# PacificBiosciences/pb-StarPhase

Hardware: AMD Instinct MI355X
Metric: HiFi reads/sec diplotyped (HLA+CYP2D6) (higher is better)
Workload: dtype int32; 1 GPU; BASELINE configs[1] + configs[2] as ONE sample per step: HLA-A/-B 10000 HiFi reads vs IMGT/HLA v0.14.1 (11,199 DNA alleles) + CYP2D6 2000 targeted reads (39 templates), the six configs[2] scenarios in turn; a new sample uploaded every step; reads -> diplotypes; hla_reads=10000, cyp2d6_reads=2000, cyp2d6_lanes=6, hla_lanes=2, cyp2d6_consensus=launch pairs

## Files before the change

### pb-starphase_amd/csrc/sp_api.hip

```cpp
#include "sp_internal.h"
#include <algorithm>
#include <thread>
#include <atomic>
#include <cstring>
#include <new>
#include <unistd.h>

extern "C" {

int32_t sp_abi_version(void) { return SP_ABI_VERSION; }

int32_t sp_device_count(int32_t* count) {
    int n = 0;
    hipError_t e = hipGetDeviceCount(&n);
    if (count) *count = (e == hipSuccess) ? n : 0;
    return e == hipSuccess ? SP_OK : SP_ERR_NO_DEVICE;
}

int32_t sp_ctx_create(int32_t device, void* stream, sp_ctx** out) {
    if (!out) return SP_ERR_INVALID_ARG;
    *out = nullptr;
    static std::atomic<int> effective{-1};
    bool by_library = false;
    if (effective.load() < 0) {
// ... 62 lines not shown
    if (ctx->ev_fork) hipEventDestroy(ctx->ev_fork);
    if (ctx->ev_join) hipEventDestroy(ctx->ev_join);
    hipStreamSynchronize(ctx->stream);
    for (sp_seqset* s : ctx->live_sets) {
        for (void* p : { (void*)s->d_words, (void*)s->d_nplane, (void*)s->d_word_off, (void*)s->d_len, (void*)s->d_kcode, (void*)s->d_kpos, (void*)s->d_koff }) if (p) ctx->dev_cap.erase(p);
        s->ctx = nullptr;
    }
    for (auto& kv : ctx->dev_cap) (void)hipFree(kv.first);
    if (ctx->scratch) hipFree(ctx->scratch);
    for (auto& kv : ctx->pool) if (kv.second.first) hipFree(kv.second.first);
    for (auto& kv : ctx->host_pool) if (kv.second.first) hipHostFree(kv.second.first);
    sp_profile_flush(ctx);
    for (hipEvent_t e : ctx->prof_free) hipEventDestroy(e);
    if (ctx->ev0) hipEventDestroy(ctx->ev0);
    if (ctx->ev1) hipEventDestroy(ctx->ev1);
    if (ctx->own_stream && ctx->stream) hipStreamDestroy(ctx->stream);
    delete ctx;
}

}
sp_ctx* sp_ctx_helper(sp_ctx* ctx, int i) {
    if (i < 0 || i > 6) return nullptr;
    if (!ctx->helper[i] && sp_ctx_create(ctx->device, nullptr, &ctx->helper[i]) != SP_OK) ctx->helper[i] = nullptr;
    if (ctx->helper[i]) { ctx->helper[i]->profiling = ctx->profiling; ctx->helper[i]->k5_block_pairs = ctx->k5_block_pairs; ctx->helper[i]->k8_persistent = ctx->k8_persistent; ctx->helper[i]->k8_side_orders = ctx->k8_side_orders; ctx->helper[i]->k8_compound = ctx->k8_compound; ctx->helper[i]->k8_side_max_blocks = ctx->k8_side_max_blocks; ctx->helper[i]->mm2_rescore = ctx->mm2_rescore; ctx->helper[i]->profile_rescore_counts = ctx->profile_rescore_counts; ctx->helper[i]->k1_best_n = ctx->k1_best_n; }
    return ctx->helper[i];
}
void sp_profile_merge(sp_ctx* into, sp_ctx* from) {
    sp_profile_flush(from);
    for (auto& kv : from->prof) { ProfileEntry& e = into->prof[kv.first]; e.ms += kv.second.ms; e.launches += kv.second.launches; e.cells += kv.second.cells; }
    from->prof.clear();
}
extern "C" {

int32_t sp_struct_size(const char* name) {
    if (!name) return -1;
#define SP_SZ(T) if (std::strcmp(name, #T) == 0) return (int32_t)sizeof(T);
    SP_SZ(sp_ctx_info)
    SP_SZ(sp_pair)
    SP_SZ(sp_aln)
    SP_SZ(sp_hla_db_desc)
    SP_SZ(sp_hla_realign)
    SP_SZ(sp_k1_seed_hit)
    SP_SZ(sp_hla_best)
    SP_SZ(sp_chain_problem)
    SP_SZ(sp_chain_result)
    SP_SZ(sp_region_hit)
    SP_SZ(sp_cyp_problem)
// ... 36 lines not shown
    SP_SZ(sp_starphase_batch_timing)
    SP_SZ(sp_hla_alleles_stats)
    SP_SZ(sp_hla_cfg_mapping)
    SP_SZ(sp_hla_cfg_gene)
    SP_SZ(sp_pileup_col)
    SP_SZ(sp_support_summary)
    SP_SZ(sp_support_entry)
#undef SP_SZ
    return -1;
}

const char* sp_last_error(const sp_ctx* ctx) { return ctx ? ctx->err.c_str() : "null context"; }

int32_t sp_ctx_synchronize(sp_ctx* ctx) {
    if (!ctx) return SP_ERR_INVALID_ARG;
    SP_HIP_CHECK(ctx, hipStreamSynchronize(ctx->stream));
    return SP_OK;
}

int32_t sp_ctx_set_option(sp_ctx* ctx, const char* name, int64_t value) {
    if (!ctx || !name) return SP_ERR_INVALID_ARG;
    if (std::strcmp(name, "hla_split_genes") == 0) { ctx->split_genes = value != 0; return SP_OK; }
    if (std::strcmp(name, "k1_best_n") == 0) { if (value < 0 || value > 8) return sp_fail(ctx, SP_ERR_INVALID_ARG, "sp_ctx_set_option: k1_best_n is 0..8"); ctx->k1_best_n = (int)value; for (sp_ctx* h : ctx->helper) if (h) h->k1_best_n = ctx->k1_best_n; return SP_OK; }
    if (std::strcmp(name, "profile_rescore_counts") == 0) { ctx->profile_rescore_counts = value != 0; for (sp_ctx* h : ctx->helper) if (h) h->profile_rescore_counts = ctx->profile_rescore_counts; return SP_OK; }
    if (std::strcmp(name, "mm2_rescore") == 0) { ctx->mm2_rescore = (int)value; for (sp_ctx* h : ctx->helper) if (h) h->mm2_rescore = ctx->mm2_rescore; return SP_OK; }
    if (std::strcmp(name, "k8_side_orders") == 0) { if (value < 0 || value > 3) return sp_fail(ctx, SP_ERR_INVALID_ARG, "sp_ctx_set_option: k8_side_orders is 0 .. 3"); ctx->k8_side_orders = (int)value; for (sp_ctx* h : ctx->helper) if (h) h->k8_side_orders = ctx->k8_side_orders; return SP_OK; }
    if (std::strcmp(name, "k8_compound") == 0) { ctx->k8_compound = (int)value; for (sp_ctx* h : ctx->helper) if (h) h->k8_compound = ctx->k8_compound; return SP_OK; }
    if (std::strcmp(name, "k8_side_max_blocks") == 0) { if (value < 0) return sp_fail(ctx, SP_ERR_INVALID_ARG, "sp_ctx_set_option: k8_side_max_blocks >= 0"); ctx->k8_side_max_blocks = (int)value; for (sp_ctx* h : ctx->helper) if (h) h->k8_side_max_blocks = ctx->k8_side_max_blocks; return SP_OK; }
    if (std::strcmp(name, "k8_persistent") == 0) { if (value < 0 || value > 2) return sp_fail(ctx, SP_ERR_INVALID_ARG, "sp_ctx_set_option: k8_persistent is 0 (never), 1 (whenever a batch fits) or 2 (the library decides)"); ctx->k8_persistent = (int)value; ctx->k8_persist_backoff = 0; ctx->k8_persist_failures = 0; for (sp_ctx* h : ctx->helper) if (h) h->k8_persistent = ctx->k8_persistent; return SP_OK; }
    if (std::strcmp(name, "cons_retry_ladder") == 0) { ctx->cons_retry_ladder = value != 0; for (sp_ctx* h : ctx->helper) if (h) h->cons_retry_ladder = ctx->cons_retry_ladder; return SP_OK; }
    if (std::strcmp(name, "k5_block_pairs") == 0) { if (value < 0 || value > (1 << 20)) return sp_fail(ctx, SP_ERR_INVALID_ARG, "sp_ctx_set_option: k5_block_pairs is 0..1048576"); ctx->k5_block_pairs = (int)value; for (sp_ctx* h : ctx->helper) if (h) h->k5_block_pairs = ctx->k5_block_pairs; return SP_OK; }
    if (std::strcmp(name, "cyp_cohort_min_group") == 0) { if (value < 1 || value > 64) return sp_fail(ctx, SP_ERR_INVALID_ARG, "sp_ctx_set_option: cyp_cohort_min_group is 1..64"); ctx->cyp_cohort_min_group = (int)value; return SP_OK; }
    if (std::strcmp(name, "cyp_cohort_streams") == 0) { if (value < 1 || value > 8) return sp_fail(ctx, SP_ERR_INVALID_ARG, "sp_ctx_set_option: cyp_cohort_streams is 1..8"); ctx->cyp_cohort_streams = (int)value; return SP_OK; }
    if (std::strcmp(name, "hla_split_streams") == 0) { if (value < 1 || value > 4) return sp_fail(ctx, SP_ERR_INVALID_ARG, "sp_ctx_set_option: hla_split_streams is 1..4"); ctx->split_streams = (int)value; return SP_OK; }
    return sp_fail(ctx, SP_ERR_INVALID_ARG, std::string("sp_ctx_set_option: unknown option ") + name);
}

int32_t sp_profile_reset(sp_ctx* ctx) {
    if (!ctx) return SP_ERR_INVALID_ARG;
    for (sp_ctx* h : ctx->helper) if (h) sp_profile_reset(h);
    sp_profile_flush(ctx); ctx->prof.clear();
    unsigned long long* c = sp_counters(ctx);
    if (c) { hipSetDevice(ctx->device); hipMemsetAsync(c, 0, SPC_N * sizeof(unsigned long long), ctx->stream); }
    return SP_OK;
}

// ... 200 lines not shown
    ctx->dev_cap[p] = want;
    return p;
}
void sp_dev_release(sp_ctx* ctx, void* p) {
    if (!p) return;
    constexpr size_t MAX_BYTES = (size_t)2 << 30, MAX_BUFFERS = 4096;
    {
        std::lock_guard<std::mutex> g(ctx->dev_cache_mu);
        auto it = ctx->dev_cap.find(p);
        if (it == ctx->dev_cap.end()) { (void)hipFree(p); return; }
        if (ctx->dev_cache.size() < MAX_BUFFERS && ctx->dev_cache_bytes + it->second <= MAX_BYTES) { ctx->dev_cache.emplace(it->second, p); ctx->dev_cache_bytes += it->second; return; }
        ctx->dev_cap.erase(it);
    }
    (void)hipFree(p);
}
extern "C" {

int32_t sp_seqset_skipped(const sp_seqset* s, uint32_t* n_skipped) { if (!s || !n_skipped) return SP_ERR_INVALID_ARG; *n_skipped = s->n_skipped; return SP_OK; }

void sp_seqset_free(sp_seqset* s) {
    if (!s) return;
    if (s->ctx) hipSetDevice(s->ctx->device);
    if (s->up) { (void)upload_finish(s); }
    if (s->ctx) {
        (void)hipStreamSynchronize(s->ctx->stream);
        { std::lock_guard<std::mutex> g(s->ctx->dev_cache_mu); s->ctx->live_sets.erase(s); }
        sp_dev_release(s->ctx, s->d_words); sp_dev_release(s->ctx, s->d_nplane); sp_dev_release(s->ctx, s->d_word_off); sp_dev_release(s->ctx, s->d_len);
        sp_dev_release(s->ctx, s->d_kcode); sp_dev_release(s->ctx, s->d_kpos); sp_dev_release(s->ctx, s->d_koff);
    } else {
        if (s->d_words) hipFree(s->d_words);
        if (s->d_nplane) hipFree(s->d_nplane);
        if (s->d_word_off) hipFree(s->d_word_off);
        if (s->d_len) hipFree(s->d_len);
        if (s->d_kcode) hipFree(s->d_kcode);
        if (s->d_kpos) hipFree(s->d_kpos);
        if (s->d_koff) hipFree(s->d_koff);
    }
    delete s;
}

int32_t sp_seqset_count(const sp_seqset* s, uint32_t* n) { if (!s || !n) return SP_ERR_INVALID_ARG; *n = s->n; return SP_OK; }
int32_t sp_seqset_length(const sp_seqset* s, uint32_t idx, uint32_t* len) {
    if (!s || !len || idx >= s->n) return SP_ERR_INVALID_ARG;
    *len = (uint32_t)s->h_len[idx]; return SP_OK;
}

// ... 171 lines not shown
    hipMemcpy(s->d_koff, koff.data(), koff.size() * 8, hipMemcpyHostToDevice);
    s->has_index = true;
    return SP_OK;
}

extern "C" {

int32_t sp_anchor_batch_topk(sp_ctx* ctx, const sp_seqset* A, const sp_seqset* B,
                             const uint32_t* a_idx, const uint32_t* b_idx, uint64_t n_pairs, int32_t topk,
                             int32_t* diag_out, int32_t* votes_out) {
    if (!ctx || !A || !B || (n_pairs && (!a_idx || !b_idx || !diag_out || !votes_out))) return SP_ERR_INVALID_ARG;
    if (topk < 1 || topk > 8) return sp_fail(ctx, SP_ERR_INVALID_ARG, "anchor: topk must be 1..8");
    if (n_pairs == 0) return SP_OK;
    hipSetDevice(ctx->device);
    for (uint64_t i = 0; i < n_pairs; ++i) if (a_idx[i] >= A->n || b_idx[i] >= B->n) return sp_fail(ctx, SP_ERR_INVALID_ARG, "anchor: index out of range");
    int rc = sp_seqset_build_index(ctx, const_cast<sp_seqset*>(A));
    if (rc) return rc;
    const size_t nb = n_pairs * 4, nbk = nb * (size_t)topk;
    uint32_t* d_a = (uint32_t*)sp_pool(ctx, "anchor_a", nb); uint32_t* d_b = (uint32_t*)sp_pool(ctx, "anchor_b", nb);
    int32_t* d_d = (int32_t*)sp_pool(ctx, "anchor_d", nbk); int32_t* d_v = (int32_t*)sp_pool(ctx, "anchor_v", nbk);
    if (!d_a || !d_b || !d_d || !d_v) return sp_fail(ctx, SP_ERR_OUT_OF_MEMORY, "anchor buffers");
    hipMemcpyAsync(d_a, a_idx, nb, hipMemcpyHostToDevice, ctx->stream);
    hipMemcpyAsync(d_b, b_idx, nb, hipMemcpyHostToDevice, ctx->stream);
    rc = sp_launch_anchor(ctx, A, B, d_a, d_b, n_pairs, d_d, d_v, topk);
    if (rc == SP_OK) {
        hipMemcpyAsync(diag_out, d_d, nbk, hipMemcpyDeviceToHost, ctx->stream);
        hipMemcpyAsync(votes_out, d_v, nbk, hipMemcpyDeviceToHost, ctx->stream);
        if (hipStreamSynchronize(ctx->stream) != hipSuccess) rc = sp_fail(ctx, SP_ERR_HIP, "anchor: stream sync failed");
    }
    return rc;
}

int32_t sp_anchor_batch(sp_ctx* ctx, const sp_seqset* A, const sp_seqset* B,
                        const uint32_t* a_idx, const uint32_t* b_idx, uint64_t n_pairs,
                        int32_t* diag_out, int32_t* votes_out) {
    return sp_anchor_batch_topk(ctx, A, B, a_idx, b_idx, n_pairs, 1, diag_out, votes_out);
}

int32_t sp_align_batch(sp_ctx* ctx, const sp_seqset* A, const sp_seqset* B,
                       const sp_pair* pairs, uint64_t n_pairs,
                       sp_aln* out, uint32_t* events, uint32_t events_stride) {
    if (!ctx || !A || !B || (n_pairs && (!pairs || !out))) return SP_ERR_INVALID_ARG;
    if (events && (events_stride == 0 || events_stride > SP_MAX_ED)) return sp_fail(ctx, SP_ERR_INVALID_ARG, "align: events_stride must be 1..SP_MAX_ED");
    if (n_pairs == 0) return SP_OK;
    hipSetDevice(ctx->device);
    std::vector<CellDesc> cells(n_pairs);
    for (uint64_t i = 0; i < n_pairs; ++i) {
// ... 24 lines not shown
```

### pb-starphase_amd/csrc/sp_cyp.hip

```cpp
#include "sp_internal.h"
#include <system_error>
#include <thread>
#include <atomic>
#include <memory>
#include <map>
#include "sp_json.h"
#include "sp_wfa.hip.h"
#include <algorithm>
#include <cmath>
#include <cstring>
#include <numeric>
#include <string>
#include <vector>

namespace {

inline bool t_is_cyp2d(int t) { return t == SP_CYP_CYP2D6 || t == SP_CYP_CYP2D7 || t == SP_CYP_DELETION || t == SP_CYP_HYBRID; }
inline bool t_is_rep(int t) { return t == SP_CYP_REP6 || t == SP_CYP_REP7; }
inline bool t_is_reported(int t) { return t == SP_CYP_CYP2D6 || t == SP_CYP_DELETION || t == SP_CYP_HYBRID; }
inline bool t_allowed(int t) { return t != SP_CYP_UNKNOWN && t != SP_CYP_FALSE_ALLELE; }
inline bool t_normalizing(int t, bool all) { return all ? t_is_cyp2d(t) : t == SP_CYP_CYP2D6; }
inline bool t_head(int t, bool all) {
    if (t == SP_CYP_REP6 || t == SP_CYP_DELETION) return true;
    if (t == SP_CYP_CYP2D6 || t == SP_CYP_HYBRID) return t_normalizing(t, all);
// ... 591 lines not shown
    if (e != hipSuccess) return sp_fail(ctx, SP_ERR_HIP, std::string("cyp placements: ") + hipGetErrorString(e));
    return SP_OK;
}

__global__ void cyp_all_pairs_kernel(uint32_t nA, uint64_t n_pairs, uint32_t* __restrict__ a_idx, uint32_t* __restrict__ b_idx) {
    const uint64_t i = (uint64_t)blockIdx.x * blockDim.x + threadIdx.x;
    if (i >= n_pairs) return;
    a_idx[i] = (uint32_t)(i % nA); b_idx[i] = (uint32_t)(i / nA);
}
static int cyp_align_all_pinned(sp_ctx* ctx, const sp_seqset* A, const sp_seqset* B, int topk, double frac_cap, const char* prof, sp_aln** out, int32_t** diag_out, int32_t** votes_out) {
    const uint64_t nA = A->n, n_pairs = nA * (uint64_t)B->n, n_cells = n_pairs * (uint64_t)topk;
    *out = nullptr; *diag_out = nullptr; *votes_out = nullptr;
    if (n_pairs == 0) return SP_OK;
    int rc = sp_seqset_build_index(ctx, const_cast<sp_seqset*>(A));
    if (rc) return rc;
    uint32_t* d_a = (uint32_t*)sp_pool(ctx, "cyp_a", n_pairs * 4); uint32_t* d_b = (uint32_t*)sp_pool(ctx, "cyp_b", n_pairs * 4);
    int32_t* d_d = (int32_t*)sp_pool(ctx, "cyp_d", n_cells * 4); int32_t* d_v = (int32_t*)sp_pool(ctx, "cyp_v", n_cells * 4);
    CellDesc* d_cells = (CellDesc*)sp_pool(ctx, "cyp_cells", n_cells * sizeof(CellDesc));
    sp_aln* d_alns = (sp_aln*)sp_pool(ctx, "cyp_alns", n_cells * sizeof(sp_aln));
    sp_aln* h_alns = (sp_aln*)sp_host_pool(ctx, "k3_alns_host", n_cells * sizeof(sp_aln));
    int32_t* h_d = (int32_t*)sp_host_pool(ctx, "k3_diag_host", n_cells * 4); int32_t* h_v = (int32_t*)sp_host_pool(ctx, "k3_votes_host", n_cells * 4);
    if (!d_a || !d_b || !d_d || !d_v || !d_cells || !d_alns || !h_alns || !h_d || !h_v) return sp_fail(ctx, SP_ERR_OUT_OF_MEMORY, "cyp placement buffers");
    hipLaunchKernelGGL(cyp_all_pairs_kernel, dim3((unsigned)((n_pairs + 255) / 256)), dim3(256), 0, ctx->stream, (uint32_t)nA, n_pairs, d_a, d_b);
    rc = sp_launch_anchor(ctx, A, B, d_a, d_b, n_pairs, d_d, d_v, topk, "anchor", (uint32_t)nA);
    if (rc) return rc;
    hipLaunchKernelGGL(cyp_build_cells_kernel, dim3((unsigned)((n_cells + 255) / 256)), dim3(256), 0, ctx->stream, d_a, d_b, d_d, d_v, n_pairs, topk, CYP_MIN_VOTES, A->d_len, frac_cap, d_cells);
    rc = sp_launch_cells(ctx, A, B, d_cells, n_cells, d_alns, nullptr, 0, prof, 0);
    if (rc) return rc;
    (void)hipMemcpyAsync(h_alns, d_alns, n_cells * sizeof(sp_aln), hipMemcpyDeviceToHost, ctx->stream);
    (void)hipMemcpyAsync(h_d, d_d, n_cells * 4, hipMemcpyDeviceToHost, ctx->stream);
    (void)hipMemcpyAsync(h_v, d_v, n_cells * 4, hipMemcpyDeviceToHost, ctx->stream);
    hipError_t e = hipStreamSynchronize(ctx->stream);
    if (e != hipSuccess) return sp_fail(ctx, SP_ERR_HIP, std::string("cyp placements: ") + hipGetErrorString(e));
    *out = h_alns; *diag_out = h_d; *votes_out = h_v;
    return SP_OK;
}

static int cyp_align_all(sp_ctx* ctx, const sp_seqset* A, const sp_seqset* B, int topk, double frac_cap, int retry_wide, const char* prof, std::vector<sp_aln>& out,
                         std::vector<int32_t>* diag_out = nullptr, std::vector<int32_t>* votes_out = nullptr) {
    const uint64_t nA = A->n, nB = B->n, n_pairs = nA * nB;
    std::vector<uint32_t> ai(n_pairs), bi(n_pairs);
    for (uint64_t b = 0; b < nB; ++b) for (uint64_t a = 0; a < nA; ++a) { ai[b * nA + a] = (uint32_t)a; bi[b * nA + a] = (uint32_t)b; }
    return cyp_align_pairs(ctx, A, B, ai, bi, (uint32_t)nA, topk, frac_cap, retry_wide, prof, out, diag_out, votes_out);
}

static inline double cyp_score(int seq_len, int nm, int unmapped, bool penalize) {
    const int len = penalize ? seq_len : seq_len - unmapped;
// ... 1303 lines not shown
                                             sp_cyp_region_variants* region_variants) {
    return spi_cyp_diplotype_mappings(ctx, pr, reads, call, consensus, cons_cap, region_variants, nullptr);
}

extern "C" int32_t sp_cyp_diplotype_mappings(sp_ctx* ctx, const sp_cyp_problem* pr, const sp_seqset* reads, sp_cyp_call* call, char* consensus, uint32_t cons_cap,
                                             sp_cyp_region_variants* region_variants, sp_cyp_read_mapping* mappings, uint64_t cap, uint64_t* n_mappings) {
    if (!n_mappings || (cap && !mappings)) return ctx ? sp_fail(ctx, SP_ERR_INVALID_ARG, "sp_cyp_diplotype_mappings: null argument") : SP_ERR_INVALID_ARG;
    std::vector<sp_cyp_read_mapping> all;
    const int32_t rc = spi_cyp_diplotype_mappings(ctx, pr, reads, call, consensus, cons_cap, region_variants, &all);
    *n_mappings = all.size();
    if (rc != SP_OK) return rc;
    std::copy(all.begin(), all.begin() + std::min<uint64_t>(cap, all.size()), mappings);
    return all.size() > cap ? sp_fail(ctx, SP_ERR_CAPACITY, "sp_cyp_diplotype_mappings: more read mappings than cap") : SP_OK;
}

int32_t spi_cyp_diplotype_cohort_mappings(sp_ctx* ctx, const sp_cyp_problem* pr, uint32_t n_samples, const sp_seqset* const* reads, sp_cyp_call* calls,
                                          char* consensus, uint32_t cons_cap, sp_cyp_region_variants* region_variants,
                                          std::vector<sp_cyp_read_mapping>* mappings, int32_t* sample_rc) {
    if (!ctx) return SP_ERR_INVALID_ARG;
    if (!pr || (n_samples && (!reads || !calls))) return sp_fail(ctx, SP_ERR_INVALID_ARG, "sp_cyp_diplotype_cohort: null argument");
    for (uint32_t i = 0; i < n_samples; ++i) if (!reads[i]) return sp_fail(ctx, SP_ERR_INVALID_ARG, "sp_cyp_diplotype_cohort: null read set");
    if (n_samples == 0) return SP_OK;
    if (pr->templates) { const int rc0 = sp_seqset_build_index(ctx, const_cast<sp_seqset*>(pr->templates)); if (rc0 != SP_OK) return rc0; }
    const uint32_t stream_cap = ctx->k8_persistent ? std::min(ctx->cyp_cohort_streams, 4) : ctx->cyp_cohort_streams;
    int n_parts = ctx->split_genes ? (int)std::min<uint32_t>(std::max<uint32_t>(1, n_samples / (uint32_t)ctx->cyp_cohort_min_group), stream_cap) : 1;
    sp_ctx* on[8] = { ctx, nullptr, nullptr, nullptr, nullptr, nullptr, nullptr, nullptr };
    for (int x = 1; x < n_parts; ++x) { on[x] = sp_ctx_helper(ctx, x - 1); if (!on[x]) { n_parts = x; break; } }
    std::vector<int32_t> rcs(n_samples, SP_OK); std::vector<int> where(n_samples, 0);
    std::atomic<uint32_t> next(0);
    const uint32_t group = std::min<uint32_t>(64, std::max<uint32_t>(1, (n_samples + (uint32_t)n_parts - 1) / (uint32_t)n_parts));
    auto work = [&](int x) {
        sp_ctx* c = on[x];
        (void)hipSetDevice(c->device);
        for (;;) {
            const uint32_t first = next.fetch_add(group);
            if (first >= n_samples) break;
            const uint32_t n = std::min<uint32_t>(group, n_samples - first);
            std::vector<std::unique_ptr<CypMid>> mids(n);
            std::vector<sp_priority_job> jobs; std::vector<uint32_t> job_of;
            try {
                std::vector<std::vector<sp_region_hit>> group_hits; int32_t rc_regions = SP_OK;
                sp_seqset view; std::vector<uint32_t> view_first;
                const bool viewed = pr->templates && pr->template_type && cyp_group_view(c, reads + first, n, "cypg", view, view_first, rc_regions);
                const bool searched = viewed && (rc_regions != SP_OK || cyp_group_regions(c, pr, view, view_first, n, group_hits, rc_regions));
                for (uint32_t k = 0; k < n; ++k) {
                    const uint32_t i = first + k;
// ... 255 lines not shown
```

### pb-starphase_amd/csrc/sp_internal.h

```cpp
#pragma once
#include <hip/hip_runtime.h>
#include <stdint.h>
#include <string>
#include <vector>
#include <chrono>
#include <set>
#include <mutex>
#include <map>
#include "../../include/starphase_hip.h"

#define SP_NEG        (-(1 << 28))
#define SP_SEQ_PAD_WORDS 512
#define SP_LDS_TAIL    288
#define SP_WAVE       64
#define SP_MAXOCC     4
#define SP_CELL_NONE  0xFFFFFFFFu
#define SP_PEAK_SPREAD   48
#define SP_PEAK_SUPPRESS 128

struct SeqSetView {
    const uint32_t* words;
    const uint32_t* nplane;
    const uint64_t* word_off;
    const int32_t*  len;
// ... 4 lines not shown
    const uint32_t* code;
    const int32_t*  pos;
    const uint64_t* off;
};

struct sp_seqset {
    sp_ctx* ctx = nullptr;
    uint32_t n = 0;
    bool has_n = false;
    std::vector<int32_t>  h_len;
    std::vector<uint64_t> h_word_off;
    std::vector<uint32_t> h_words;
    uint32_t* d_words = nullptr;
    uint32_t* d_nplane = nullptr;
    uint64_t* d_word_off = nullptr;
    int32_t*  d_len = nullptr;
    int32_t   max_len = 0;
    uint32_t  n_skipped = 0;
    struct sp_upload* up = nullptr;
    int32_t up_rc = 0; std::string up_err;
    bool has_index = false;
    uint32_t* d_kcode = nullptr; int32_t* d_kpos = nullptr; uint64_t* d_koff = nullptr;
    SeqSetView view() const { return SeqSetView{d_words, d_nplane, d_word_off, d_len, n}; }
    KmerIndexView kview() const { return KmerIndexView{d_kcode, d_kpos, d_koff}; }
};

struct ProfileEntry { double ms = 0; uint64_t launches = 0; uint64_t cells = 0; };

struct sp_ctx {
    int device = 0;
    hipStream_t stream = nullptr;
    bool own_stream = false;
    std::string err;
    bool profiling = true;
    hipEvent_t ev0 = nullptr, ev1 = nullptr;
    std::map<std::string, ProfileEntry> prof;
    struct PendingProf { hipEvent_t e0, e1; const char* name; uint64_t cells; };
    std::vector<PendingProf> prof_pending;
    std::vector<hipEvent_t> prof_free;
    void* scratch = nullptr; size_t scratch_bytes = 0;
    std::map<std::string, std::pair<void*, size_t>> pool;
    uint64_t pool_allocs = 0;
    std::map<std::string, std::pair<void*, size_t>> host_pool;
    std::multimap<size_t, void*> dev_cache; std::map<void*, size_t> dev_cap; size_t dev_cache_bytes = 0; std::mutex dev_cache_mu;
    std::set<sp_seqset*> live_sets;
    int num_cus = 256;
    int hw_queues = 4; bool hw_queues_by_library = false; std::string warning;
    bool split_genes = true;
    int split_streams = 3;
    bool cons_retry_ladder = false;
    hipStream_t copy_stream = nullptr;
    hipStream_t ctl_stream = nullptr;
    hipEvent_t ev_fork = nullptr, ev_join = nullptr;
    int k1_best_n = 5;
    int profile_rescore_counts = 0;
    int mm2_rescore = 1;
    int k8_persistent = 2;
    int hw_queues_effective = 0;
    int k8_side_orders = 1;
    int k8_compound = 1;
    int k8_side_max_blocks = 4096;
    int k8_persist_backoff = 0;
    int k8_persist_failures = 0;
    sp_seqset* uploading = nullptr;
    int k5_block_pairs = 4096;
    int cyp_cohort_min_group = 12;
    int cyp_cohort_streams = 8;
    sp_ctx* helper[7] = { nullptr, nullptr, nullptr, nullptr, nullptr, nullptr, nullptr };
};

struct CellDesc {
    uint32_t a, b;
    int32_t  diag;
    int32_t  max_ed;
    int32_t  b_lo, b_hi;
};

// ... 20 lines not shown
};
int  sp_k1_seed_build(sp_ctx* ctx, const sp_seqset* alleles, K1Seed** out);
void sp_k1_seed_free(K1Seed* s);
void sp_k1_seed_stats(const K1Seed* s, int64_t out[4]);
int  sp_k1_seed_sketch(sp_ctx* ctx, const sp_seqset* set, uint32_t idx, uint64_t* hash, int32_t* end_pos, uint8_t* strand, uint32_t cap, uint32_t* n_out);
int  sp_k1_seed_map(sp_ctx* ctx, const K1Seed* idx, const sp_seqset* alleles, const sp_seqset* reads, int best_n, int32_t* d_best, sp_k1_seed_info* d_info,
                    sp_aln* d_win_aln, sp_affine_aln* d_win_af, const K1SeedDebug* dbg, sp_hla_rev_hit* d_rev = nullptr);

sp_ctx* sp_ctx_helper(sp_ctx* ctx, int i = 0);
void sp_profile_merge(sp_ctx* into, sp_ctx* from);
int sp_launch_anchor(sp_ctx* ctx, const sp_seqset* A, const sp_seqset* B,
                     const uint32_t* d_a_idx, const uint32_t* d_b_idx, uint64_t n_pairs,
                     int32_t* d_diag, int32_t* d_votes, int topk = 1, const char* prof_name = "anchor", uint32_t a_period = 1);
int sp_launch_cells(sp_ctx* ctx, const sp_seqset* A, const sp_seqset* B,
                    const CellDesc* d_cells, uint64_t n_cells,
                    sp_aln* d_out, uint32_t* d_events, uint32_t events_stride, const char* prof_name, int retry_wide = 0);

int sp_launch_affine(sp_ctx* ctx, const sp_seqset* A, const sp_seqset* B, const void* d_pairs , uint64_t n_pairs, const sp_affine_opts& o, int band,
                     sp_affine_aln* d_out, const char* prof_name, const uint32_t* d_n_live = nullptr, const void* d_wins = nullptr, const void* d_mids = nullptr);
int sp_rescore_mappings(sp_ctx* ctx, const sp_seqset* Aw, const sp_seqset* Bw, const CellDesc* d_cells, const sp_aln* d_ref, uint64_t n, bool target_is_a,
                        const sp_affine_opts& o, int band, sp_affine_aln* d_out, const char* prefix, uint32_t stride, int trace_retry_wide = 0, const sp_aln* d_tr_in = nullptr, const uint32_t* d_ev_in = nullptr, int ends_only = 0, int windows = -1, void* d_audit = nullptr);
int sp_launch_affine_map(sp_ctx* ctx, const sp_seqset* A, const sp_seqset* B, const void* d_pairs , uint64_t n_pairs, const sp_affine_opts& o, sp_affine_aln* d_out,
                         uint32_t* d_n_cigar, uint64_t* d_op_off, uint32_t* d_ops, uint64_t ops_cap, unsigned long long* d_cursor, const char* prof_name);
constexpr uint32_t SP_ANCHOR_SKIP = 0xFFFFFFFFu;
int sp_launch_cells_wide(sp_ctx* ctx, const sp_seqset* A, const sp_seqset* B, const CellDesc* d_cells, uint64_t n_cells, sp_aln* d_out);
int sp_launch_pack_on(hipStream_t stream, int num_cus, int format, const void* d_src, const uint64_t* d_off, const uint64_t* d_word_off, const int32_t* d_len, uint32_t n,
                      uint32_t* d_words, uint32_t* d_nplane, uint32_t* d_flag);
int sp_launch_pack(sp_ctx* ctx, const char* d_ascii, const uint64_t* d_off, const uint64_t* d_word_off, const int32_t* d_len, uint32_t n,
                   uint32_t* d_words, uint32_t* d_nplane, uint32_t* d_flag);
int sp_make_segments(sp_ctx* ctx, const sp_seqset* reads, const std::vector<uint32_t>& idx, const std::vector<int32_t>& start,
                     const std::vector<int32_t>& len, const char* prefix, sp_seqset* seg, sp_seqset* hpc);
int sp_seqset_make_small(sp_ctx* ctx, const char* prefix, const char* bases, const uint64_t* offsets, uint32_t n, bool with_index, sp_seqset* out);
int sp_seqset_fetch_host(sp_ctx* ctx, sp_seqset* s);
std::string sp_seqset_decode(sp_ctx* ctx, const sp_seqset* s, uint32_t i);
enum { SPC_K1_ACTIVE = 0, SPC_K1_EXECUTED, SPC_K1_RESUMED, SPC_K1_BYTES, SPC_CONS_LAUNCHES, SPC_CONS_COLUMNS, SPC_N = 16 };
unsigned long long* sp_counters(sp_ctx* ctx);
void* sp_scratch(sp_ctx* ctx, size_t bytes);
void* sp_pool(sp_ctx* ctx, const char* name, size_t bytes);
size_t sp_pool_bytes(const sp_ctx* ctx, const char* name);
void* sp_host_pool(sp_ctx* ctx, const char* name, size_t bytes);
int   sp_fail(sp_ctx* ctx, int code, const std::string& msg);
#define SP_HIP_CHECK(ctx, expr) do { hipError_t _e = (expr); if (_e != hipSuccess) \
    return sp_fail((ctx), SP_ERR_HIP, std::string(#expr) + ": " + hipGetErrorString(_e)); } while (0)

void sp_profile_flush(sp_ctx* ctx);
struct HostMarks {
// ... 37 lines not shown
```

Measured before the change: 353,300 reads/s.

## Add k-mer dictionary anchor voting for CYP2D6 template placement

Builds a per-template-set dictionary of the distinct template k-mers plus a dense per-template hit table, then maps each read k-mer to a dictionary id once per read. The anchor kernel then looks up hits by direct table index instead of searching each template's k-mer index for every read/template pair. This is on by default for the CYP2D6 region search and opt-in for batch top-k. It costs a one-time host build and device memory of nA×D words, and falls back to the old kernel when that exceeds a budget.

```diff
diff --git a/pb-starphase_amd/csrc/sp_anchor_dict.hip b/pb-starphase_amd/csrc/sp_anchor_dict.hip
--- /dev/null
+++ b/pb-starphase_amd/csrc/sp_anchor_dict.hip
@@ -0,0 +1,231 @@
+#include "sp_internal.h"
+#include "sp_wfa.hip.h"
+#include "sp_anchor.hip.h"
+#include "sp_anchor_dict_host.h"
+#include <algorithm>
+#include <cstdlib>
+#include <mutex>
+
+constexpr size_t SP_ADICT_BUDGET_BYTES = (size_t)256 << 20;
+constexpr size_t SP_ADICT_IDS_CAP_BYTES = (size_t)64 << 20;
+#ifndef SP_ADICT_BUCKET_BITS
+#define SP_ADICT_BUCKET_BITS 16
+#endif
+#ifndef SP_ADICT_THREADS
+#define SP_ADICT_THREADS 256
+#endif
+#ifndef SP_ADICT_WG_PER_CU
+#define SP_ADICT_WG_PER_CU 8
+#endif
+#ifndef SP_ADICT_AHEAD
+#define SP_ADICT_AHEAD 4
+#endif
+#ifndef SP_ADICT_TABPOS
+#define SP_ADICT_TABPOS 0
+#endif
+
+struct sp_anchor_dict {
+    bool built = false;
+    size_t need_bytes = 0;
+    uint32_t D = 0;
+    uint32_t* d_code = nullptr; uint32_t* d_bucket = nullptr; uint32_t* d_hits = nullptr;
+};
+static std::mutex g_adict_mu;
+
+static size_t env_bytes(const char* name, size_t dflt) {
+    const char* v = std::getenv(name);
+    if (!v || !*v) return dflt;
+    char* end = nullptr; const unsigned long long x = std::strtoull(v, &end, 10);
+    return end && end != v ? (size_t)x : dflt;
+}
+
+void sp_anchor_dict_free(sp_seqset* A) {
+    if (!A || !A->adict) return;
+    sp_anchor_dict* d = A->adict;
+    if (A->ctx) { sp_dev_release(A->ctx, d->d_code); sp_dev_release(A->ctx, d->d_bucket); sp_dev_release(A->ctx, d->d_hits); }
+    else { if (d->d_code) (void)hipFree(d->d_code); if (d->d_bucket) (void)hipFree(d->d_bucket); if (d->d_hits) (void)hipFree(d->d_hits); }
+    delete d; A->adict = nullptr;
+}
+
+int sp_anchor_dict_build(sp_ctx* ctx, sp_seqset* A) {
+    if (!A->has_index) return sp_fail(ctx, SP_ERR_INVALID_ARG, "anchor dictionary: set A has no k-mer index");
+    const size_t budget = env_bytes("SP_ANCHOR_DICT_BUDGET", SP_ADICT_BUDGET_BYTES);
+    std::lock_guard<std::mutex> g(g_adict_mu);
+    if (!A->adict) { A->adict = new (std::nothrow) sp_anchor_dict(); if (!A->adict) return sp_fail(ctx, SP_ERR_OUT_OF_MEMORY, "anchor dictionary"); }
+    sp_anchor_dict* d = A->adict;
+    if (d->need_bytes && d->need_bytes > budget) return SP_ANCHOR_DICT_REFUSED;
+    if (d->built) return SP_OK;
+    (void)hipSetDevice(ctx->device);
+    const auto t0 = std::chrono::steady_clock::now();
+    std::vector<uint64_t> koff((size_t)A->n + 1, 0);
+    if (hipMemcpy(koff.data(), A->d_koff, koff.size() * 8, hipMemcpyDeviceToHost) != hipSuccess) return sp_fail(ctx, SP_ERR_HIP, "anchor dictionary: fetch table offsets");
+    std::vector<uint32_t> kcode((size_t)koff[A->n]);
+    if (!kcode.empty() && hipMemcpy(kcode.data(), A->d_kcode, kcode.size() * 4, hipMemcpyDeviceToHost) != hipSuccess) return sp_fail(ctx, SP_ERR_HIP, "anchor dictionary: fetch codes");
+    AnchorDictHost h;
+    if (!anchor_dict_host_build(A->n, koff.data(), kcode.data(), SP_ADICT_BUCKET_BITS, SP_MAXOCC, &h)) { d->need_bytes = SIZE_MAX; return SP_ANCHOR_DICT_REFUSED; }
+    d->need_bytes = std::max<size_t>(4, h.hits.size() * 4);
+    if (d->need_bytes > budget) return SP_ANCHOR_DICT_REFUSED;
+    sp_ctx* owner = A->ctx ? A->ctx : ctx;
+    auto up = [&](const std::vector<uint32_t>& v, uint32_t** dst) {
+        *dst = (uint32_t*)(A->ctx ? sp_dev_alloc(owner, std::max<size_t>(1, v.size()) * 4) : nullptr);
+        if (!A->ctx && hipMalloc(dst, std::max<size_t>(1, v.size()) * 4) != hipSuccess) *dst = nullptr;
+        if (!*dst) return false;
+        return v.empty() || hipMemcpy(*dst, v.data(), v.size() * 4, hipMemcpyHostToDevice) == hipSuccess;
+    };
+    if (!up(h.code, &d->d_code) || !up(h.bucket, &d->d_bucket) || !up(h.hits, &d->d_hits)) return sp_fail(ctx, SP_ERR_OUT_OF_MEMORY, "anchor dictionary: device buffers");
+    d->D = (uint32_t)h.code.size(); d->built = true;
+    if (ctx->profiling) {
+        auto& e = ctx->prof["host:anchor_dict_build"];
+        e.ms += std::chrono::duration<double, std::milli>(std::chrono::steady_clock::now() - t0).count(); e.launches += 1; e.cells += d->D;
+    }
+    return SP_OK;
+}
+
+__global__ __launch_bounds__(256) void sp_anchor_ids_kernel(SeqSetView B, uint32_t b0, uint32_t b1, const uint64_t* __restrict__ id_off, uint64_t off0, const uint32_t* __restrict__ code,
+                                                             const uint32_t* __restrict__ bucket, uint32_t D, uint32_t* __restrict__ ids) {
+    for (uint32_t b = b0 + blockIdx.x; b < b1; b += gridDim.x) {
+        const int n = B.len[b];
+        const uint64_t woff = B.word_off[b];
+        const uint32_t* bw = B.words + woff;
+        const uint32_t* bn = B.nplane ? B.nplane + woff : nullptr;
+        uint32_t* out = ids + (id_off[b] - off0);
+        for (int j = threadIdx.x; j < n; j += 256) {
+            bool ok = j + SP_KMER <= n;
+            const int w = ok ? j >> 4 : 0; const uint32_t sh = (uint32_t)((j & 15) << 1);
+            if (ok && bn && __builtin_amdgcn_alignbit(bn[w + 1], bn[w], sh)) ok = false;
+            uint32_t id = 0xFFFFFFFFu;
+            if (ok) {
+                const uint32_t c = __builtin_amdgcn_alignbit(bw[w + 1], bw[w], sh);
+                const uint32_t q = c >> (32 - SP_ADICT_BUCKET_BITS);
+                uint32_t lo = bucket[q], hi = bucket[q + 1];
+                while (lo < hi) { const uint32_t mid = (lo + hi) >> 1; if (code[mid] < c) lo = mid + 1; else hi = mid; }
+                if (lo < D && code[lo] == c) id = lo;
+            }
+            out[j] = id;
+        }
+    }
+}
+
+template <int THREADS, bool TABPOS>
+__global__ __launch_bounds__(THREADS) void sp_anchor_dict_kernel(SeqSetView A, KmerIndexView KA, SeqSetView B, const uint32_t* __restrict__ a_idx, const uint32_t* __restrict__ b_idx,
+                                                                 uint64_t p_begin, uint64_t p_end, uint32_t b0, uint32_t b1, int first_batch,
+                                                                 const uint32_t* __restrict__ ids, const uint64_t* __restrict__ id_off, uint64_t off0, const uint32_t* __restrict__ hits, uint32_t D,
+                                                                 int32_t* __restrict__ diag_out, int32_t* __restrict__ votes_out, int bins_cap, int topk, int tab_cap) {
+    extern __shared__ uint32_t lds[];
+    __shared__ unsigned long long red[THREADS / 64];
+    __shared__ int spread[2];
+    constexpr int AHEAD = SP_ADICT_AHEAD;
+    const int tid = threadIdx.x;
+    int32_t* tab_pos = reinterpret_cast<int32_t*>(lds + ((bins_cap + 1) >> 1));
+    int tab_a = -1;
+    for (uint64_t p = p_begin + blockIdx.x; p < p_end; p += gridDim.x) {
+        const uint32_t a = a_idx[p], b = b_idx[p];
+        if (b == SP_ANCHOR_SKIP) {
+            if (first_batch && tid == 0) for (int k2 = 0; k2 < topk; ++k2) { diag_out[p * topk + k2] = 0; votes_out[p * topk + k2] = 0; }
+            continue;
+        }
+        if (b < b0 || b >= b1) continue;
+        const int m = A.len[a], n = B.len[b];
+        const int nbins = m + n + 1;
+        if (m < SP_KMER || n < SP_KMER || nbins > bins_cap) {
+            if (tid == 0) for (int k2 = 0; k2 < topk; ++k2) { diag_out[p * topk + k2] = 0; votes_out[p * topk + k2] = 0; }
+            continue;
+        }
+        const int nb32 = (nbins + 1) >> 1;
+        const uint32_t* my_ids = ids + (id_off[b] - off0);
+        const uint32_t* my_hits = hits + (size_t)a * D;
+        const uint64_t k0 = KA.off[a]; const int nk = (int)(KA.off[a + 1] - k0);
+        uint32_t hv[AHEAD];
+        auto load = [&](int base) {
+#pragma unroll
+            for (int u = 0; u < AHEAD; ++u) { const int j = base + u * THREADS + tid; hv[u] = j + SP_KMER <= n ? my_ids[j] : 0xFFFFFFFFu; }
+#pragma unroll
+            for (int u = 0; u < AHEAD; ++u) hv[u] = hv[u] != 0xFFFFFFFFu ? my_hits[hv[u]] : 0u;
+        };
+        load(0);
+        sp_anchor_clear<THREADS>(lds, nb32);
+        const bool in_lds = TABPOS && nk <= tab_cap;
+        if (in_lds && (int)a != tab_a) { for (int i = tid; i < nk; i += THREADS) tab_pos[i] = KA.pos[k0 + i]; }
+        tab_a = in_lds ? (int)a : -1;
+        const int32_t* kp = in_lds ? tab_pos : KA.pos + k0;
+        __syncthreads();
+        for (int base = 0; base + SP_KMER <= n; base += AHEAD * THREADS) {
+            int pos1[AHEAD];
+#pragma unroll
+            for (int u = 0; u < AHEAD; ++u) pos1[u] = (hv[u] >> 24) ? kp[hv[u] & 0xFFFFFFu] : 0;
+#pragma unroll
+            for (int u = 0; u < AHEAD; ++u) {
+                const int j = base + u * THREADS + tid;
+                const int cnt = (int)(hv[u] >> 24), first = (int)(hv[u] & 0xFFFFFFu);
+                sp_anchor_vote_run(lds, cnt == 1 ? j - pos1[u] + m : -1);
+                if (cnt > 1)
+                    for (int y = 0; y < cnt; ++y) {
+                        const int bin = j - kp[first + y] + m;
+                        atomicAdd(&lds[bin >> 1], (bin & 1) ? 0x10000u : 1u);
+                    }
+            }
+            if (base + AHEAD * THREADS + SP_KMER <= n) load(base + AHEAD * THREADS);
+        }
+        __syncthreads();
+        sp_anchor_peaks<THREADS>(lds, nbins, m, topk, p, diag_out, votes_out, red, spread);
+        __syncthreads();
+    }
+}
+
+int sp_launch_anchor_dict(sp_ctx* ctx, const sp_seqset* A, const sp_seqset* B, const uint32_t* d_a_idx, const uint32_t* d_b_idx, const uint32_t* h_b_idx, uint64_t n_pairs,
+                          uint32_t grid_nA, int32_t* d_diag, int32_t* d_votes, int topk, const char* prof_name) {
+    if (topk < 1 || topk > 8) return sp_fail(ctx, SP_ERR_INVALID_ARG, "anchor: topk must be 1..8");
+    if (n_pairs == 0) return SP_OK;
+    if (!A->has_index) return sp_fail(ctx, SP_ERR_INVALID_ARG, "anchor: set A has no k-mer index");
+    if ((size_t)((A->max_len + B->max_len + 2) / 2) * 4 > 160 * 1024 - 64) return sp_fail(ctx, SP_ERR_TOO_LONG, "anchor: sequences too long for the LDS vote histogram");
+    if (B->n == 0 || (grid_nA == 0 && !h_b_idx)) return SP_ANCHOR_DICT_REFUSED;
+    const int rc = sp_anchor_dict_build(ctx, const_cast<sp_seqset*>(A));
+    if (rc != SP_OK) return rc;
+    const sp_anchor_dict* d = A->adict;
+    (void)hipSetDevice(ctx->device);
+    uint32_t lo = 0, hi = B->n;
+    if (grid_nA == 0) { lo = B->n; hi = 0; for (uint64_t i = 0; i < n_pairs; ++i) if (h_b_idx[i] != SP_ANCHOR_SKIP) { lo = std::min(lo, h_b_idx[i]); hi = std::max(hi, h_b_idx[i] + 1); } if (lo >= hi) { lo = 0; hi = 1; } }
+    const size_t cap_slots = std::max<size_t>(1, env_bytes("SP_ANCHOR_IDS_CAP", SP_ADICT_IDS_CAP_BYTES) / 4);
+    uint64_t* h_off = (uint64_t*)sp_host_pool(ctx, "anchor_idoff_host", ((size_t)B->n + 1) * 8);
+    uint64_t* d_off = (uint64_t*)sp_pool(ctx, "anchor_idoff", ((size_t)B->n + 1) * 8);
+    if (!h_off || !d_off) return sp_fail(ctx, SP_ERR_OUT_OF_MEMORY, "anchor: id offsets");
+    h_off[0] = 0;
+    for (uint32_t b = 0; b < B->n; ++b) h_off[b + 1] = h_off[b] + (uint64_t)((std::max(B->h_len[b], 0) + 3) & ~3);
+    struct Batch { uint32_t b0, b1; int max_len; };
+    std::vector<Batch> batches; size_t most_slots = 0;
+    for (uint32_t b0 = lo; b0 < hi;) {
+        uint32_t b1 = b0 + 1; int ml = B->h_len[b0];
+        while (b1 < hi && h_off[b1 + 1] - h_off[b0] <= cap_slots) { ml = std::max(ml, B->h_len[b1]); ++b1; }
+        batches.push_back(Batch{b0, b1, ml}); most_slots = std::max<size_t>(most_slots, h_off[b1] - h_off[b0]);
+        b0 = b1;
+    }
+    uint32_t* d_ids = (uint32_t*)sp_pool(ctx, "anchor_ids", std::max<size_t>(4, most_slots * 4));
+    if (!d_ids) return sp_fail(ctx, SP_ERR_OUT_OF_MEMORY, "anchor: ids buffer");
+    SP_HIP_CHECK(ctx, hipMemcpyAsync(d_off, h_off, ((size_t)B->n + 1) * 8, hipMemcpyHostToDevice, ctx->stream));
+    const SeqSetView av = A->view(), bv = B->view(); const KmerIndexView kv = A->kview();
+    auto* kern = sp_anchor_dict_kernel<SP_ADICT_THREADS, SP_ADICT_TABPOS != 0>;
+    for (size_t x = 0; x < batches.size(); ++x) {
+        const Batch& bt = batches[x];
+        const uint64_t off0 = h_off[bt.b0];
+        {
+            ProfScope ps(ctx, "anchor_ids", bt.b1 - bt.b0);
+            const unsigned grid = std::min<unsigned>(bt.b1 - bt.b0, (unsigned)ctx->num_cus * 8);
+            hipLaunchKernelGGL(sp_anchor_ids_kernel, dim3(grid), dim3(256), 0, ctx->stream, bv, bt.b0, bt.b1, (const uint64_t*)d_off, off0, d->d_code, d->d_bucket, d->D, d_ids);
+            SP_HIP_CHECK(ctx, hipGetLastError());
+        }
+        const int bins_cap = A->max_len + bt.max_len + 1;
+        size_t lds_bytes = (size_t)((bins_cap + 1) / 2) * 4;
+        int tab_cap = SP_ADICT_TABPOS ? A->max_len : 0;
+        if (lds_bytes + (size_t)tab_cap * 4 > 160 * 1024 - 64) tab_cap = 0;
+        lds_bytes += (size_t)tab_cap * 4;
+        const uint64_t p_begin = grid_nA ? (uint64_t)bt.b0 * grid_nA : 0, p_end = grid_nA ? (uint64_t)bt.b1 * grid_nA : n_pairs;
+        uint64_t grid = std::min<uint64_t>(p_end - p_begin, (uint64_t)ctx->num_cus * SP_ADICT_WG_PER_CU);
+        if (SP_ADICT_TABPOS && grid_nA > 1 && grid > grid_nA) grid -= grid % grid_nA;
+        SP_HIP_CHECK(ctx, hipFuncSetAttribute((const void*)kern, hipFuncAttributeMaxDynamicSharedMemorySize, (int)lds_bytes));
+        ProfScope ps(ctx, prof_name, p_end - p_begin);
+        hipLaunchKernelGGL(kern, dim3((unsigned)grid), dim3(SP_ADICT_THREADS), lds_bytes, ctx->stream, av, kv, bv, d_a_idx, d_b_idx, p_begin, p_end, bt.b0, bt.b1, x == 0 ? 1 : 0,
+                           (const uint32_t*)d_ids, (const uint64_t*)d_off, off0, (const uint32_t*)d->d_hits, d->D, d_diag, d_votes, bins_cap, topk, tab_cap);
+        SP_HIP_CHECK(ctx, hipGetLastError());
+    }
+    return SP_OK;
+}
diff --git a/pb-starphase_amd/csrc/sp_anchor_dict_host.h b/pb-starphase_amd/csrc/sp_anchor_dict_host.h
--- /dev/null
+++ b/pb-starphase_amd/csrc/sp_anchor_dict_host.h
@@ -0,0 +1,35 @@
+#pragma once
+#include <stdint.h>
+#include <algorithm>
+#include <vector>
+
+struct AnchorDictHost {
+    std::vector<uint32_t> code;
+    std::vector<uint32_t> bucket;
+    std::vector<uint32_t> hits;
+};
+
+inline bool anchor_dict_host_build(uint32_t nA, const uint64_t* koff, const uint32_t* kcode, int bucket_bits, int max_occ, AnchorDictHost* out) {
+    out->code.clear(); out->bucket.clear(); out->hits.clear();
+    for (uint32_t a = 0; a < nA; ++a) if (koff[a + 1] - koff[a] >= (1ull << 24)) return false;
+    out->code.assign(kcode, kcode + koff[nA]);
+    std::sort(out->code.begin(), out->code.end());
+    out->code.erase(std::unique(out->code.begin(), out->code.end()), out->code.end());
+    const size_t D = out->code.size();
+    const uint32_t nb = 1u << bucket_bits; const int sh = 32 - bucket_bits;
+    out->bucket.assign((size_t)nb + 1, 0);
+    for (size_t i = 0; i < D; ++i) ++out->bucket[(out->code[i] >> sh) + 1];
+    for (uint32_t q = 0; q < nb; ++q) out->bucket[q + 1] += out->bucket[q];
+    out->hits.assign((size_t)nA * D, 0u);
+    for (uint32_t a = 0; a < nA; ++a) {
+        size_t id = 0;
+        for (uint64_t i = koff[a]; i < koff[a + 1];) {
+            uint64_t e = i + 1;
+            while (e < koff[a + 1] && kcode[e] == kcode[i]) ++e;
+            while (out->code[id] < kcode[i]) ++id;
+            if (e - i <= (uint64_t)max_occ) out->hits[(size_t)a * D + id] = (uint32_t)(i - koff[a]) | (uint32_t)(e - i) << 24;
+            i = e;
+        }
+    }
+    return true;
+}
diff --git a/pb-starphase_amd/csrc/sp_api.hip b/pb-starphase_amd/csrc/sp_api.hip
--- a/pb-starphase_amd/csrc/sp_api.hip
+++ b/pb-starphase_amd/csrc/sp_api.hip
@@ -108,7 +108,7 @@
 sp_ctx* sp_ctx_helper(sp_ctx* ctx, int i) {
     if (i < 0 || i > 6) return nullptr;
     if (!ctx->helper[i] && sp_ctx_create(ctx->device, nullptr, &ctx->helper[i]) != SP_OK) ctx->helper[i] = nullptr;
-    if (ctx->helper[i]) { ctx->helper[i]->profiling = ctx->profiling; ctx->helper[i]->k5_block_pairs = ctx->k5_block_pairs; ctx->helper[i]->k8_persistent = ctx->k8_persistent; ctx->helper[i]->k8_side_orders = ctx->k8_side_orders; ctx->helper[i]->k8_compound = ctx->k8_compound; ctx->helper[i]->k8_side_max_blocks = ctx->k8_side_max_blocks; ctx->helper[i]->mm2_rescore = ctx->mm2_rescore; ctx->helper[i]->profile_rescore_counts = ctx->profile_rescore_counts; ctx->helper[i]->k1_best_n = ctx->k1_best_n; }
+    if (ctx->helper[i]) { ctx->helper[i]->profiling = ctx->profiling; ctx->helper[i]->k5_block_pairs = ctx->k5_block_pairs; ctx->helper[i]->k8_persistent = ctx->k8_persistent; ctx->helper[i]->k8_side_orders = ctx->k8_side_orders; ctx->helper[i]->k8_compound = ctx->k8_compound; ctx->helper[i]->k8_side_max_blocks = ctx->k8_side_max_blocks; ctx->helper[i]->mm2_rescore = ctx->mm2_rescore; ctx->helper[i]->profile_rescore_counts = ctx->profile_rescore_counts; ctx->helper[i]->k1_best_n = ctx->k1_best_n; ctx->helper[i]->anchor_dict = ctx->anchor_dict; }
     return ctx->helper[i];
 }
 void sp_profile_merge(sp_ctx* into, sp_ctx* from) {
@@ -191,6 +191,7 @@
     if (!ctx || !name) return SP_ERR_INVALID_ARG;
     if (std::strcmp(name, "hla_split_genes") == 0) { ctx->split_genes = value != 0; return SP_OK; }
     if (std::strcmp(name, "k1_best_n") == 0) { if (value < 0 || value > 8) return sp_fail(ctx, SP_ERR_INVALID_ARG, "sp_ctx_set_option: k1_best_n is 0..8"); ctx->k1_best_n = (int)value; for (sp_ctx* h : ctx->helper) if (h) h->k1_best_n = ctx->k1_best_n; return SP_OK; }
+    if (std::strcmp(name, "anchor_dict") == 0) { if (value < 0 || value > 2) return sp_fail(ctx, SP_ERR_INVALID_ARG, "sp_ctx_set_option: anchor_dict is 0 (never), 1 (the CYP2D6 region search) or 2 (sp_anchor_batch_topk too)"); ctx->anchor_dict = (int)value; for (sp_ctx* h : ctx->helper) if (h) h->anchor_dict = ctx->anchor_dict; return SP_OK; }
     if (std::strcmp(name, "profile_rescore_counts") == 0) { ctx->profile_rescore_counts = value != 0; for (sp_ctx* h : ctx->helper) if (h) h->profile_rescore_counts = ctx->profile_rescore_counts; return SP_OK; }
     if (std::strcmp(name, "mm2_rescore") == 0) { ctx->mm2_rescore = (int)value; for (sp_ctx* h : ctx->helper) if (h) h->mm2_rescore = ctx->mm2_rescore; return SP_OK; }
     if (std::strcmp(name, "k8_side_orders") == 0) { if (value < 0 || value > 3) return sp_fail(ctx, SP_ERR_INVALID_ARG, "sp_ctx_set_option: k8_side_orders is 0 .. 3"); ctx->k8_side_orders = (int)value; for (sp_ctx* h : ctx->helper) if (h) h->k8_side_orders = ctx->k8_side_orders; return SP_OK; }
@@ -437,6 +438,7 @@
     if (!s) return;
     if (s->ctx) hipSetDevice(s->ctx->device);
     if (s->up) { (void)upload_finish(s); }
+    sp_anchor_dict_free(s);
     if (s->ctx) {
         (void)hipStreamSynchronize(s->ctx->stream);
         { std::lock_guard<std::mutex> g(s->ctx->dev_cache_mu); s->ctx->live_sets.erase(s); }
@@ -654,7 +656,8 @@
     if (!d_a || !d_b || !d_d || !d_v) return sp_fail(ctx, SP_ERR_OUT_OF_MEMORY, "anchor buffers");
     hipMemcpyAsync(d_a, a_idx, nb, hipMemcpyHostToDevice, ctx->stream);
     hipMemcpyAsync(d_b, b_idx, nb, hipMemcpyHostToDevice, ctx->stream);
-    rc = sp_launch_anchor(ctx, A, B, d_a, d_b, n_pairs, d_d, d_v, topk);
+    rc = ctx->anchor_dict >= 2 ? sp_launch_anchor_dict(ctx, A, B, d_a, d_b, b_idx, n_pairs, 0, d_d, d_v, topk, "anchor") : SP_ANCHOR_DICT_REFUSED;
+    if (rc == SP_ANCHOR_DICT_REFUSED) rc = sp_launch_anchor(ctx, A, B, d_a, d_b, n_pairs, d_d, d_v, topk);
     if (rc == SP_OK) {
         hipMemcpyAsync(diag_out, d_d, nbk, hipMemcpyDeviceToHost, ctx->stream);
         hipMemcpyAsync(votes_out, d_v, nbk, hipMemcpyDeviceToHost, ctx->stream);
diff --git a/pb-starphase_amd/csrc/sp_cyp.hip b/pb-starphase_amd/csrc/sp_cyp.hip
--- a/pb-starphase_amd/csrc/sp_cyp.hip
+++ b/pb-starphase_amd/csrc/sp_cyp.hip
@@ -637,7 +637,8 @@
     int32_t* h_d = (int32_t*)sp_host_pool(ctx, "k3_diag_host", n_cells * 4); int32_t* h_v = (int32_t*)sp_host_pool(ctx, "k3_votes_host", n_cells * 4);
     if (!d_a || !d_b || !d_d || !d_v || !d_cells || !d_alns || !h_alns || !h_d || !h_v) return sp_fail(ctx, SP_ERR_OUT_OF_MEMORY, "cyp placement buffers");
     hipLaunchKernelGGL(cyp_all_pairs_kernel, dim3((unsigned)((n_pairs + 255) / 256)), dim3(256), 0, ctx->stream, (uint32_t)nA, n_pairs, d_a, d_b);
-    rc = sp_launch_anchor(ctx, A, B, d_a, d_b, n_pairs, d_d, d_v, topk, "anchor", (uint32_t)nA);
+    rc = ctx->anchor_dict >= 1 ? sp_launch_anchor_dict(ctx, A, B, d_a, d_b, nullptr, n_pairs, (uint32_t)nA, d_d, d_v, topk, "anchor") : SP_ANCHOR_DICT_REFUSED;
+    if (rc == SP_ANCHOR_DICT_REFUSED) rc = sp_launch_anchor(ctx, A, B, d_a, d_b, n_pairs, d_d, d_v, topk, "anchor", (uint32_t)nA);
     if (rc) return rc;
     hipLaunchKernelGGL(cyp_build_cells_kernel, dim3((unsigned)((n_cells + 255) / 256)), dim3(256), 0, ctx->stream, d_a, d_b, d_d, d_v, n_pairs, topk, CYP_MIN_VOTES, A->d_len, frac_cap, d_cells);
     rc = sp_launch_cells(ctx, A, B, d_cells, n_cells, d_alns, nullptr, 0, prof, 0);
@@ -1987,6 +1988,7 @@
     for (uint32_t i = 0; i < n_samples; ++i) if (!reads[i]) return sp_fail(ctx, SP_ERR_INVALID_ARG, "sp_cyp_diplotype_cohort: null read set");
     if (n_samples == 0) return SP_OK;
     if (pr->templates) { const int rc0 = sp_seqset_build_index(ctx, const_cast<sp_seqset*>(pr->templates)); if (rc0 != SP_OK) return rc0; }
+    if (pr->templates && ctx->anchor_dict >= 1) { const int rc0 = sp_anchor_dict_build(ctx, const_cast<sp_seqset*>(pr->templates)); if (rc0 != SP_OK && rc0 != SP_ANCHOR_DICT_REFUSED) return rc0; }
     const uint32_t stream_cap = ctx->k8_persistent ? std::min(ctx->cyp_cohort_streams, 4) : ctx->cyp_cohort_streams;
     int n_parts = ctx->split_genes ? (int)std::min<uint32_t>(std::max<uint32_t>(1, n_samples / (uint32_t)ctx->cyp_cohort_min_group), stream_cap) : 1;
     sp_ctx* on[8] = { ctx, nullptr, nullptr, nullptr, nullptr, nullptr, nullptr, nullptr };
diff --git a/pb-starphase_amd/csrc/sp_internal.h b/pb-starphase_amd/csrc/sp_internal.h
--- a/pb-starphase_amd/csrc/sp_internal.h
+++ b/pb-starphase_amd/csrc/sp_internal.h
@@ -50,6 +50,7 @@
     bool has_index = false;
     uint32_t* d_kcode = nullptr; int32_t* d_kpos = nullptr; uint64_t* d_koff = nullptr;
     SeqSetView view() const { return SeqSetView{d_words, d_nplane, d_word_off, d_len, n}; }
+    struct sp_anchor_dict* adict = nullptr;
     KmerIndexView kview() const { return KmerIndexView{d_kcode, d_kpos, d_koff}; }
 };
 
@@ -81,6 +82,7 @@
     hipStream_t ctl_stream = nullptr;
     hipEvent_t ev_fork = nullptr, ev_join = nullptr;
     int k1_best_n = 5;
+    int anchor_dict = 1;
     int profile_rescore_counts = 0;
     int mm2_rescore = 1;
     int k8_persistent = 2;
@@ -147,6 +149,11 @@
                         const sp_affine_opts& o, int band, sp_affine_aln* d_out, const char* prefix, uint32_t stride, int trace_retry_wide = 0, const sp_aln* d_tr_in = nullptr, const uint32_t* d_ev_in = nullptr, int ends_only = 0, int windows = -1, void* d_audit = nullptr);
 int sp_launch_affine_map(sp_ctx* ctx, const sp_seqset* A, const sp_seqset* B, const void* d_pairs , uint64_t n_pairs, const sp_affine_opts& o, sp_affine_aln* d_out,
                          uint32_t* d_n_cigar, uint64_t* d_op_off, uint32_t* d_ops, uint64_t ops_cap, unsigned long long* d_cursor, const char* prof_name);
+constexpr int SP_ANCHOR_DICT_REFUSED = 1;
+int sp_launch_anchor_dict(sp_ctx* ctx, const sp_seqset* A, const sp_seqset* B, const uint32_t* d_a_idx, const uint32_t* d_b_idx, const uint32_t* h_b_idx, uint64_t n_pairs,
+                          uint32_t grid_nA, int32_t* d_diag, int32_t* d_votes, int topk, const char* prof_name);
+int  sp_anchor_dict_build(sp_ctx* ctx, sp_seqset* A);
+void sp_anchor_dict_free(sp_seqset* A);
 constexpr uint32_t SP_ANCHOR_SKIP = 0xFFFFFFFFu;
 int sp_launch_cells_wide(sp_ctx* ctx, const sp_seqset* A, const sp_seqset* B, const CellDesc* d_cells, uint64_t n_cells, sp_aln* d_out);
 int sp_launch_pack_on(hipStream_t stream, int num_cus, int format, const void* d_src, const uint64_t* d_off, const uint64_t* d_word_off, const int32_t* d_len, uint32_t n,
```

Measured after the change: 352,500 reads/s. No clear change (-0.2%).
